# xxlong0/NeuralUDF

Measured on AMD Instinct MI355X. Metric: ray-samples/sec (train step), higher is better.
Workload: dtype f32 emulated on the 16-bit matrix pipe, f32 accumulate, f32 state / epilogues / optimizer.  Forward-order sweeps (UDF value, input gradient, colour / NeRF forward): f16x2 (x = hi + 2^-11 lo in fp16, 3 fp16 MFMA products, correction terms in their own accumulator).  Backward sweeps (tangent, adjoint

## Files before the change

### include/nudf.h

```cpp
#ifndef NUDF_H
#define NUDF_H
#include <stdint.h>

#ifdef __cplusplus
extern "C" {
#endif

int nudf_version(void);
const char* nudf_last_error(void);

enum {
  NUDF_STATUS_NONFINITE_RENDER = 1,
  NUDF_STATUS_NONFINITE_SAMPLES = 2,
  NUDF_STATUS_NONFINITE_LOSS = 4
};
int nudf_set_status_flag(int32_t* device_word);
int32_t* nudf_status_flag(void);

enum {
  NUDF_EPI_NONE = 0,
  NUDF_EPI_SOFTPLUS = 1,
  NUDF_EPI_RELU = 2,
  NUDF_EPI_MUL = 3,
  NUDF_EPI_MULMASK = 4,
// ... 375 lines not shown
  const float* seed_wrow;
  unsigned long long* dbg;
  float* absmax_out;
  const float* tile_amax_in;
  float* tile_amax_out;
  int32_t tile_scale;
  int32_t reserved0;
  NudfChainStep step[NUDF_CH_MAX_STEPS];
} NudfChain;
#if defined(__cplusplus)
static_assert(sizeof(NudfChain) <= 4096, "NudfChain travels by value: the kernel-argument segment holds 4 KB");
#endif
int nudf_mlp_chain(const NudfChain* args, void* stream);
int nudf_chain_max_steps(void);
int nudf_set_chain_t16(int on);
int nudf_pack_frag(const float* B, int ldb, int K, int N, float* out, void* stream);

#define NUDF_PACK_MAX_LAYERS 16
#define NUDF_PACK_MAX_FRAGS 4
typedef struct NudfPackFrag {
  float* dst;
  int32_t transpose;
  int32_t o0, i0;
  int32_t K, N;
  int32_t dtype;
} NudfPackFrag;
typedef struct NudfPackLayer {
  const float* v; const float* g;
  const int32_t* perm;
  float* W; float* Wt;
// ... 196 lines not shown
```

### neuraludf_amd/_lib.py

```python
from __future__ import annotations

import ctypes as C
import os

import torch

_HERE = os.path.dirname(os.path.abspath(__file__))
LIB_PATH = os.environ.get("NUDF_LIB") or os.path.join(_HERE, "libnudf.so")
ABI_VERSION = 108

c_fp = C.c_void_p
i32 = C.c_int32
f32 = C.c_float


class NudfError(RuntimeError):
    pass


class GemmNN(C.Structure):
    _fields_ = [("A", c_fp), ("lda", i32), ("B", c_fp), ("ldb", i32), ("bias", c_fp),
                ("C1", c_fp), ("ldc1", i32), ("C2", c_fp), ("ldc2", i32), ("C3", c_fp), ("ldc3", i32),
                ("X1", c_fp), ("ldx1", i32), ("X2", c_fp), ("ldx2", i32),
                ("M", i32), ("N", i32), ("K", i32), ("epi", i32), ("iparam", i32), ("scale", f32), ("xscale", f32)]
# ... 192 lines not shown

LW = dict(color_base=0, color=1, color_pixel=2, color_patch=3, igr=4, igr_ns=5, sparse=6, mask=7, color_sum=8)
LW_COUNT = 16

EPI = dict(NONE=0, SOFTPLUS=1, RELU=2, MUL=3, MULMASK=4, TANGENT=5, BWD=6, SIGMOID=7, UDFHEAD=8,
           SKIPSPLIT=9, RELU_DUAL=10, ADDMASK=11, MULSP=12)

SYMBOLS = [
    "nudf_version", "nudf_chain_max_steps", "nudf_last_error", "nudf_set_status_flag", "nudf_status_flag", "nudf_gemm_nn", "nudf_set_gemm_variant", "nudf_gemm_tn", "nudf_gemm_tn_grouped", "nudf_gemm_tn_grouped_workspace", "nudf_gemm_tn_grouped_plan", "nudf_set_tn_flags", "nudf_patch_metric", "nudf_set_tn_debug", "nudf_composite_fwd",
    "nudf_composite_bwd", "nudf_partial_sums", "nudf_composite_colour_finish", "nudf_set_composite_blocked", "nudf_upsample", "nudf_merge", "nudf_merge_points", "nudf_coarse_z", "nudf_coarse_start", "nudf_outside_z",
    "nudf_ray_points", "nudf_posenc", "nudf_posenc_vjp", "nudf_copy_cols", "nudf_add_cols",
    "nudf_udf_grad_seed", "nudf_udf_head_bwd", "nudf_signed_colsum", "nudf_sigmoid_head_bwd",
    "nudf_weightnorm_pack", "nudf_weightnorm_unpack_grad",
    "nudf_pixel_blend_fwd", "nudf_pixel_blend_bwd", "nudf_pixel_composite_fwd", "nudf_pixel_composite_bwd",
    "nudf_patch_blend_fwd", "nudf_patch_blend_bwd", "nudf_ssim_patch", "nudf_pixel_warp", "nudf_patch_warp",
    "nudf_adam_step", "nudf_adam_chunk", "nudf_mlp_chain", "nudf_set_chain_t16", "nudf_pack_frag",
    "nudf_weightnorm_pack_multi", "nudf_weightnorm_unpack_grad_multi",
    "nudf_scalars_fwd", "nudf_scalars_bwd", "nudf_l1_sum_fwd", "nudf_l1_sum_bwd",
    "nudf_sums_errors_fwd", "nudf_sums_errors_bwd", "nudf_color_loss_fwd", "nudf_color_loss_bwd",
    "nudf_gen_ray_batch", "nudf_color_loss_sums", "nudf_color_loss_finish",
    "nudf_step_loss_fwd", "nudf_step_loss_bwd", "nudf_col0_seed4",
    "nudf_blend_loss_prepare", "nudf_blend_loss_fwd", "nudf_blend_loss_bwd",
    "nudf_meshudf_classify", "nudf_meshudf_emit", "nudf_meshudf_vertices",
    "nudf_pc_tri_count", "nudf_pc_tri_emit", "nudf_pc_keys", "nudf_pc_cells", "nudf_pc_thin_round", "nudf_pc_nearest",
    "nudf_meshtopo_edges", "nudf_meshtopo_fill_count", "nudf_meshtopo_fill_emit", "nudf_meshtopo_smooth",
    "nudf_meshtopo_cc_hook", "nudf_meshtopo_cc_jump", "nudf_meshtopo_views",
]

_P, _I, _F = C.c_void_p, C.c_int, C.c_float
_ARGTYPES = {
    "nudf_gemm_nn": [C.POINTER(GemmNN), _P],
# ... 91 lines not shown
        _lib.nudf_version.restype = C.c_int
        _lib.nudf_adam_chunk.restype = C.c_int
        if _lib.nudf_version() != ABI_VERSION:
            v, _lib = _lib.nudf_version(), None
            raise NudfError(f"{LIB_PATH} is ABI version {v}, this package binds {ABI_VERSION}: rebuild with "
                            "`python -m neuraludf_amd.build --force`")
        steps = getattr(_lib, "nudf_chain_max_steps", None)
        if steps is None or int(steps()) != CH_MAX_STEPS:
            v, _lib = (None if steps is None else int(steps())), None
            raise NudfError(f"{LIB_PATH} holds {v} chain steps per launch, this package binds {CH_MAX_STEPS}: rebuild with "
                            "`python -m neuraludf_amd.build --force`")
        _bind(_lib)
        _lib.nudf_gemm_tn_grouped_workspace.restype = C.c_int64
        _lib.nudf_set_chain_t16.argtypes = [C.c_int]
        _lib.nudf_set_chain_t16.restype = C.c_int
        _lib.nudf_set_status_flag.argtypes = [C.c_void_p]
        _lib.nudf_set_status_flag.restype = C.c_int
        _lib.nudf_status_flag.argtypes = []
        _lib.nudf_status_flag.restype = C.c_void_p
    return _lib


STATUS_NONFINITE_RENDER, STATUS_NONFINITE_SAMPLES, STATUS_NONFINITE_LOSS = 1, 2, 4
_STATUS_WORDS = {}
_STATUS_BOUND = None


def bind_status(dev):
    global _STATUS_BOUND
    if dev.type != "cuda":
# ... 66 lines not shown
```

### neuraludf_amd/csrc/mlp_chain.hip

```cpp
#include "nudf_common.h"
#include "../../include/nudf.h"

#include "mlp_chain_shared.h"
#include <stdlib.h>
#include <type_traits>

template <int TM>
struct ChainSmem {
  float act[TM * CH_LD];
  float xs[TM * 3];
  float vs[TM * 3];
  float red[8];
};
#define CH_SGN_COL 288
static_assert(CH_SGN_COL < CH_LD, "the head multiplier lives in the tile's row padding");

template <int TM>
struct ChainSmem16 {
  unsigned short act[TM * CH_LD16];
  float xs[TM * 3];
  float vs[TM * 3];
  float red[8];
};

// ... 513 lines not shown
    mfmas(pa[1], b[1]);
    split(pa[0]);
    pattern();
  }
  __builtin_amdgcn_sched_barrier(0);
  if (g < G16) mfmas(pa[0], b[0]);
  }
#pragma unroll
  for (int i = 0; i < NRT; ++i)
#pragma unroll
    for (int j = 0; j < NCT; ++j)
#pragma unroll
      for (int r = 0; r < 16; ++r) acc[i][j][r] = __builtin_fmaf(acc1[i][j][r], 1.0f / 2048.0f, acc[i][j][r]);
}

typedef __bf16 ch_bf16x2 __attribute__((ext_vector_type(2)));
typedef float ch_f32x2 __attribute__((ext_vector_type(2)));
__device__ __forceinline__ void ch_p4_widen(const uint2& w, float* x) {
  x[0] = __builtin_bit_cast(float, w.x << 16);
  x[1] = __builtin_bit_cast(float, w.x & 0xffff0000u);
  x[2] = __builtin_bit_cast(float, w.y << 16);
  x[3] = __builtin_bit_cast(float, w.y & 0xffff0000u);
}
__device__ __forceinline__ void ch_p4_load(const float* X, int ld, unsigned q0, unsigned col, uint2 (&w)[4]) {
  const uint2* Xq = reinterpret_cast<const uint2*>(X) + (size_t)q0 * ld + col;
#pragma unroll
  for (int g = 0; g < 4; ++g) w[g] = Xq[(size_t)(2 * g) * ld];
}
__device__ __forceinline__ void ch_p4_store(float* C, int ld, unsigned q0, unsigned col, const float (&v)[16]) {
  uint2* Cq = reinterpret_cast<uint2*>(C) + (size_t)q0 * ld + col;
#pragma unroll
  for (int g = 0; g < 4; ++g) {
    uint2 w;
    w.x = __builtin_bit_cast(unsigned, __builtin_convertvector(ch_f32x2{v[4 * g], v[4 * g + 1]}, ch_bf16x2));
    w.y = __builtin_bit_cast(unsigned, __builtin_convertvector(ch_f32x2{v[4 * g + 2], v[4 * g + 3]}, ch_bf16x2));
    Cq[(size_t)(2 * g) * ld] = w;
  }
}

struct ChNoX3 {};
template <int EPI, bool X2IN = false, bool S16 = false, bool RT16 = false, bool T16 = false, bool HX3 = false, class X3V = ChNoX3>
__device__ __forceinline__ float ch_epilogue_tile(const NudfChainStep& st, float* act, int m0, int rtile, int ctile,
                                                 int h, int ln, f32x16 a, float (&x1)[16], bool load_x1,
                                                 const float* x2in = nullptr, const float* bias_pre = nullptr,
                                                 bool tile_bf = false, const X3V& x3in = X3V(), float tsig = 1.0f,
                                                 float tinv = 1.0f) {
  float tmax = 0.0f;
  const int col = ctile * 32 + ln;
  const bool col_ok = col < st.N;
  const unsigned colc = col_ok ? col : 0;
  const int r0 = rtile * 32 + 4 * h;
  const unsigned grow0 = (unsigned)(m0 + r0);
  float v[16], out[16];
  {
    const float bias = bias_pre ? *bias_pre : (st.bias ? st.bias[colc] : 0.0f);
#pragma unroll
    for (int r = 0; r < 16; ++r) v[r] = a[r] + bias;
  }
  if (st.r1_row) {
    const float r1c = st.r1_col[colc];
    const unsigned vo = grow0 * (unsigned)st.ldr1;
#pragma unroll
    for (int r = 0; r < 16; ++r) {
      const float rv = (st.r1_row + (size_t)CH_KOFF(r) * st.ldr1)[vo];
      tmax = fmaxf(tmax, fabsf(rv));
      v[r] += (rv * tsig) * r1c;
    }
  }
  float x2[16];
  if (CH_USES_X1(EPI) && load_x1) {
    const unsigned vo = grow0 * (unsigned)st.ldx1 + colc;
    if (S16 || (RT16 && (st.layout & NUDF_CH_P4_X1))) {
      uint2 w[4];
      ch_p4_load(st.X1, st.ldx1, (grow0 >> 2), colc, w);
// ... 128 lines not shown
#pragma unroll
          for (int r = 0; r < 16; ++r) (st.C1 + (size_t)CH_KOFF(r) * st.ldc1)[vo] = out[r];
        }
        if (st.C2 && st.N <= st.iparam) {
          const unsigned vo = grow0 * (unsigned)st.ldc2 + col;
#pragma unroll
          for (int r = 0; r < 16; ++r) (st.C2 + (size_t)CH_KOFF(r) * st.ldc2)[vo] = out[r];
        }
      } else if (st.C2) {
        const unsigned vo = grow0 * (unsigned)st.ldc2 + (col - st.iparam);
#pragma unroll
        for (int r = 0; r < 16; ++r) (st.C2 + (size_t)CH_KOFF(r) * st.ldc2)[vo] = out2[r];
      }
    }
  } else if (col_ok) {
    if (st.C1) {
      float omax = 0.0f;
#pragma unroll
      for (int r = 0; r < 16; r += 2) omax = __builtin_fmaxf(omax, __builtin_fmaxf(fabsf(out[r]), fabsf(out[r + 1])));
      tmax = __builtin_fmaxf(tmax, omax * tinv);
    }
    if (EPI == NUDF_CH_MULSP && st.iparam > 0 && col >= st.iparam) {
      if (st.C2) {
        const unsigned vo = grow0 * (unsigned)st.ldc2 + (col - st.iparam);
#pragma unroll
        for (int r = 0; r < 16; ++r) (st.C2 + (size_t)CH_KOFF(r) * st.ldc2)[vo] = out2[r] * tinv;
      }
    } else if (st.C1) {
      const unsigned vo = grow0 * (unsigned)st.ldc1 + col;
      if (S16 || (RT16 && (st.layout & NUDF_CH_P4_C1))) {
        ch_p4_store(st.C1, st.ldc1, (grow0 >> 2), (unsigned)col, out);
// ... 237 lines not shown
      for (int r = 0; r < 8; ++r) (st.C1 + (size_t)CH_KOFF(r) * st.ldc1)[vo] = out[r] * tinv;
      float omax = 0.0f;
#pragma unroll
      for (int r = 0; r < 8; r += 2) omax = __builtin_fmaxf(omax, __builtin_fmaxf(fabsf(out[r]), fabsf(out[r + 1])));
      bmax = __builtin_fmaxf(bmax, omax * tinv);
    }
    if (st.act_write) {
      float* ap = act + ((rt0 + i) * 32 + 4 * h + 16 * hf) * CH_LD + st.act_col0 + col;
#pragma unroll
      for (int r = 0; r < 8; ++r) ap[CH_KOFF(r) * CH_LD] = col_ok ? out[r] : 0.0f;
    }
  }
  return bmax;
}

template <int EPI, int MODE>
__device__ __forceinline__ float ch_epilogue(const NudfChain& p, const NudfChainStep& st, float* act, int m0, int rt0,
                                            int ct0, int nrt, int nct, int h, int ln, f32x16 (&acc)[2][2],
                                            const float (&px1)[2][2][16], const float (&bpre)[2], bool tile_bf = false,
                                            float tsig = 1.0f, float tinv = 1.0f) {
  float emax = 0.0f;
  constexpr bool ANY16 = MODE == 1 || MODE == 3 || MODE == 4, X3 = MODE == 2, T16 = MODE == 3 || MODE == 4;
  constexpr bool PF = CH_USES_X1(EPI);
  if constexpr (CH_USES_X2(EPI) && !T16) {
    if (!X3 && st.prec == 0 && nrt == 2 && !(ANY16 && (st.layout & NUDF_CH_STATE16))) {
      float(&x1)[2][2][16] = const_cast<float(&)[2][2][16]>(px1);
      if (nct == 2) ch_epilogue_seq<EPI, 2, 2>(st, act, m0, rt0, ct0, h, ln, acc, x1, bpre);
      else ch_epilogue_seq<EPI, 2, 1>(st, act, m0, rt0, ct0, h, ln, acc, x1, bpre);
      return emax;
    }
  }
// ... 73 lines not shown
            continue;
          }
        }
        ch_epilogue_tile<EPI, false, true, false, T16>(st, act, m0, rt0 + i, ct0 + j, h, ln, a, x1, true, nullptr, &bpre[j], tile_bf);
        continue;
      }
    }
    if constexpr (EPI == NUDF_CH_BWD && MODE == 1) {
      if (st.X3) {
        ch_epilogue_tile<EPI, false, false, false, T16, true>(st, act, m0, rt0 + i, ct0 + j, h, ln, a, x1, true, nullptr, &bpre[j],
                                                              tile_bf);
        continue;
      }
    }
    constexpr bool RT16 = ANY16 && (EPI == NUDF_CH_RELU || EPI == NUDF_CH_MULMASK || EPI == NUDF_CH_ADDMASK);
    emax = fmaxf(emax, ch_epilogue_tile<EPI, false, false, RT16, T16>(st, act, m0, rt0 + i, ct0 + j, h, ln, a, x1, ANY16 || X3, nullptr,
                                                                      &bpre[j], tile_bf, ChNoX3(), tsig, tinv));
  }
  return emax;
}

#ifndef NUDF_T16_WGS
#define NUDF_T16_WGS 3
#endif
#ifndef NUDF_TS_LOG2
#define NUDF_TS_LOG2 (-6)
#endif
template <int TM, int MODE>
__global__ __launch_bounds__(CH_THREADS, (MODE == 3) ? NUDF_T16_WGS : 2) void mlp_chain_kernel(NudfChain p_arg) {
  constexpr bool ANY16 = MODE == 1 || MODE == 3 || MODE == 4, X3 = MODE == 2, T16 = MODE == 3 || MODE == 4;
  (void)p_arg;
  const NudfChain& p = *(const NudfChain*)__builtin_amdgcn_kernarg_segment_ptr();
  constexpr int WMT = TM / 32;
  using Smem = typename std::conditional<T16, ChainSmem16<TM>, ChainSmem<TM>>::type;
  __shared__ __attribute__((aligned(16))) Smem sm;
  const bool tile_bf = T16 && p.step[0].prec == 2;
  const int tfmt = T16 ? (tile_bf ? 2 : 1) : 0;
  float* const act_f = reinterpret_cast<float*>(sm.act);
  const int tid = threadIdx.x;
  const int lane = tid & 63;
  const int wave = tid >> 6;
  const int h = lane >> 5, ln = lane & 31;
  const int m0 = blockIdx.x * TM;
  float amax = 0.0f;
  float tsig = 1.0f, tinv = 1.0f;
  const bool tscale = X3 && p.tile_scale != 0;
  auto wg_max = [&](float v) -> float {
#pragma unroll
    for (int off = 32; off > 0; off >>= 1) v = fmaxf(v, __shfl_xor(v, off));
    __syncthreads();
    if (lane == 0) sm.red[wave] = v;
    __syncthreads();
    float m = sm.red[0];
#pragma unroll
    for (int w = 1; w < CH_THREADS / 64; ++w) m = fmaxf(m, sm.red[w]);
    return m;
  };
  auto set_sigma = [&](float m) {
    const unsigned e = (__builtin_bit_cast(unsigned, m) >> 23) & 0xffu;
    const int se = 254 + NUDF_TS_LOG2 - (int)e;
    if (e != 0u && e != 255u && se >= 1 && se <= 254) {
// ... 5 lines not shown
    float m = 0.0f;
    for (int i = 0; i < p.n_steps; ++i) {
      const NudfChainStep& s0 = p.step[i];
      if (s0.r1_row)
        for (int e = tid; e < TM; e += CH_THREADS) m = fmaxf(m, fabsf(s0.r1_row[(size_t)min(m0 + e, p.P - 1) * s0.ldr1]));
    }
    if (p.tile_amax_in && tid < TM / 32) m = fmaxf(m, p.tile_amax_in[(m0 >> 5) + tid]);
    return m;
  };

  if (p.x) {
    for (int e = tid; e < TM * 3; e += CH_THREADS) {
      int r = m0 + e / 3;
      if (r > p.P - 1) r = p.P - 1;
      sm.xs[e] = p.x[(size_t)(r / p.x_div) * 3 + (e % 3)];
      sm.vs[e] = p.v ? p.v[(size_t)r * 3 + (e % 3)] : 0.0f;
      if (X3 && p.v && p.init == NUDF_CH_INIT_POSENC)
        amax = fmaxf(amax, fabsf(sm.vs[e] * p.pe_in_scale) * (float)(1 << (p.pe_L > 0 ? p.pe_L - 1 : 0)));
    }
  }
  if constexpr (X3) {
    if (tscale && p.init == NUDF_CH_INIT_POSENC && p.v) {
      set_sigma(wg_max(fmaxf(amax, other_seeds())));
      for (int e = tid; e < TM * 3; e += CH_THREADS) sm.vs[e] *= tsig;
    }
  }
  __syncthreads();
  if (p.init == NUDF_CH_INIT_LOAD) {
    const int k4 = p.k0 >> 2;
    for (int e = tid; e < TM * k4; e += CH_THREADS) {
      const int r = e / k4, c4 = e - r * k4;
      int gr = m0 + r;
      if (gr > p.P - 1) gr = p.P - 1;
      const f32x4 val = *reinterpret_cast<const f32x4*>(p.A0 + (size_t)gr * p.lda0 + c4 * 4);
      if constexpr (X3) amax = fmaxf(amax, fmaxf(fmaxf(fabsf(val[0]), fabsf(val[1])), fmaxf(fabsf(val[2]), fabsf(val[3]))));
      if constexpr (T16) {
        uint2 w;
        if (tile_bf) {
          w.x = (unsigned)ch_f2bf(val[0]) | ((unsigned)ch_f2bf(val[1]) << 16);
          w.y = (unsigned)ch_f2bf(val[2]) | ((unsigned)ch_f2bf(val[3]) << 16);
        } else {
          w.x = ch_f2h2(val[0], val[1]);
// ... 73 lines not shown

#ifdef NUDF_X3_CU_STAGGER
  if (X3 && gridDim.x > 256) {
    const unsigned hw = __builtin_amdgcn_s_getreg((8 << 11) | (8 << 6) | 4);
#if NUDF_X3_CU_STAGGER > 0
    const unsigned late = hw & 1u;
    for (int d = 0; d < (int)late * NUDF_X3_CU_STAGGER; ++d) __builtin_amdgcn_s_sleep(127);
#else
    const unsigned xcc = __builtin_amdgcn_s_getreg((4 << 11) | (0 << 6) | 20);
    for (int d = 0; d < (int)(xcc & 1u) * (-NUDF_X3_CU_STAGGER); ++d) __builtin_amdgcn_s_sleep(127);
#endif
  }
#endif
  unsigned long long* dbg = p.dbg ? p.dbg + ((size_t)blockIdx.x * 4 + wave) * 64 : nullptr;
  if (dbg && lane == 0) {
    dbg[0] = __builtin_amdgcn_s_getreg((31 << 11) | (0 << 6) | 4);
    dbg[1] = __builtin_amdgcn_s_memtime();
    dbg[62] = wall_clock64();
  }

  for (int si = 0; si < p.n_steps; ++si) {
    const NudfChainStep& st = p.step[si];
    if ((si + slot) & 1u) __builtin_amdgcn_s_setprio(1); else __builtin_amdgcn_s_setprio(0);
    if constexpr (X3) {
      if (st.epi == NUDF_CH_SEED) {
        int t = tid;
        asm volatile("" : "+v"(t));
        const int C = st.N;
        if (t < C) {
          const float wc = st.r1_col[t];
          float* ap = act_f + t;
          float* gp = st.C1 ? st.C1 + (size_t)m0 * st.ldc1 + t : nullptr;
#pragma unroll 4
          for (int r = 0; r < TM; ++r) {
            float s, om;
            ch_sp_derivs(ap[r * CH_LD], st.xscale, s, om);
            const float val = ap[r * CH_LD + CH_SGN_COL - t] * wc * st.scale * s;
            ap[r * CH_LD] = val;
            if (gp) gp[(size_t)r * st.ldc1] = val;
// ... 58 lines not shown
    if (nct > 0) {
      const float* arow = act_f + (rt0 * 32 + ln) * CH_LD + 4 * h;
      const f32x4* bptr = Bp + (size_t)ct0 * 64 + lane;
      const size_t bstride = (size_t)NT * 64;
      const bool pfx = !ANY16 && !X3 && CH_USES_X1(st.epi);
      ChPrefetch pf;
      pf.X1 = st.X1;
      pf.ldx1 = st.ldx1;
#pragma unroll
      for (int i = 0; i < 2; ++i)
#pragma unroll
        for (int j = 0; j < 2; ++j) {
          const int col = (ct0 + j) * 32 + ln;
          pf.vo[i][j] = (unsigned)(m0 + (rt0 + i) * 32 + 4 * h) * (unsigned)st.ldx1 + (unsigned)((col < st.N) ? col : 0);
        }
      if (X3 && st.prec == 4) {
        const float* arow16 = act_f + (rt0 * 32 + ln) * CH_LD + 8 * h;
        const uint4* bp2 = reinterpret_cast<const uint4*>(st.Bp) + (size_t)ct0 * 128 + lane;
        const size_t bstride2 = (size_t)NT * 128;
        const int G16 = st.K >> 4;
#ifdef NUDF_X2_PIPE64
        constexpr bool PIPE2 = true;
#else
        constexpr bool PIPE2 = (NUDF_X3_PIPE == 1) || (NUDF_X3_PIPE == 2 && TM == 32);
#endif
        if (nrt == 2 && nct == 2) ch_mma16x2<2, 2, PIPE2>(arow16, bp2, bstride2, G16, acc);
        else if (nrt == 2) ch_mma16x2<2, 1, PIPE2>(arow16, bp2, bstride2, G16, acc);
        else if (nct == 2) ch_mma16x2<1, 2, PIPE2>(arow16, bp2, bstride2, G16, acc);
        else ch_mma16x2<1, 1, PIPE2>(arow16, bp2, bstride2, G16, acc);
      } else if (X3 && st.prec == 3) {
// ... 30 lines not shown
        if (nrt == 2 && nct == 2) ch_mma<2, 2, true>(arow, bptr, bstride, G, acc, pf, px1);
        else if (nrt == 2) ch_mma<2, 1, true>(arow, bptr, bstride, G, acc, pf, px1);
        else if (nct == 2) ch_mma<1, 2, true>(arow, bptr, bstride, G, acc, pf, px1);
        else ch_mma<1, 1, true>(arow, bptr, bstride, G, acc, pf, px1);
      } else {
        if (nrt == 2 && nct == 2) ch_mma<2, 2, false>(arow, bptr, bstride, G, acc, pf, px1);
        else if (nrt == 2) ch_mma<2, 1, false>(arow, bptr, bstride, G, acc, pf, px1);
        else if (nct == 2) ch_mma<1, 2, false>(arow, bptr, bstride, G, acc, pf, px1);
        else ch_mma<1, 1, false>(arow, bptr, bstride, G, acc, pf, px1);
      }
    }
    if (dbg && lane == 0 && si < 14) dbg[2 + 4 * si] = __builtin_amdgcn_s_memtime();
    __syncthreads();
    if (dbg && lane == 0 && si < 14) dbg[3 + 4 * si] = __builtin_amdgcn_s_memtime();

    if (nct > 0) {
      switch (st.epi) {
        case NUDF_CH_SOFTPLUS: ch_epilogue<NUDF_CH_SOFTPLUS, MODE>(p, st, act_f, m0, rt0, ct0, nrt, nct, h, ln, acc, px1, bpre, tile_bf, tsig, tinv); break;
        case NUDF_CH_NONE: { const float em = ch_epilogue<NUDF_CH_NONE, MODE>(p, st, act_f, m0, rt0, ct0, nrt, nct, h, ln, acc, px1, bpre, tile_bf, tsig, tinv); if constexpr (X3) amax = fmaxf(amax, em); } break;
        case NUDF_CH_MULSP: { const float em = ch_epilogue<NUDF_CH_MULSP, MODE>(p, st, act_f, m0, rt0, ct0, nrt, nct, h, ln, acc, px1, bpre, tile_bf, tsig, tinv); if constexpr (X3) amax = fmaxf(amax, em); } break;
        case NUDF_CH_TANGENT:
          if constexpr (MODE != 3) ch_epilogue<NUDF_CH_TANGENT, MODE>(p, st, act_f, m0, rt0, ct0, nrt, nct, h, ln, acc, px1, bpre, tile_bf, tsig, tinv);
          break;
        case NUDF_CH_BWD: { const float em = ch_epilogue<NUDF_CH_BWD, MODE>(p, st, act_f, m0, rt0, ct0, nrt, nct, h, ln, acc, px1, bpre, tile_bf, tsig, tinv); if constexpr (X3) amax = fmaxf(amax, em); } break;
        case NUDF_CH_RELU: ch_epilogue<NUDF_CH_RELU, MODE>(p, st, act_f, m0, rt0, ct0, nrt, nct, h, ln, acc, px1, bpre, tile_bf, tsig, tinv); break;
        case NUDF_CH_SIGMOIDN: ch_epilogue<NUDF_CH_SIGMOIDN, MODE>(p, st, act_f, m0, rt0, ct0, nrt, nct, h, ln, acc, px1, bpre, tile_bf, tsig, tinv); break;
        case NUDF_CH_MULMASK: { const float em = ch_epilogue<NUDF_CH_MULMASK, MODE>(p, st, act_f, m0, rt0, ct0, nrt, nct, h, ln, acc, px1, bpre, tile_bf, tsig, tinv); if constexpr (X3) amax = fmaxf(amax, em); } break;
        case NUDF_CH_ADDMASK: { const float em = ch_epilogue<NUDF_CH_ADDMASK, MODE>(p, st, act_f, m0, rt0, ct0, nrt, nct, h, ln, acc, px1, bpre, tile_bf, tsig, tinv); if constexpr (X3) amax = fmaxf(amax, em); } break;
        case NUDF_CH_RELUADD: ch_epilogue<NUDF_CH_RELUADD, MODE>(p, st, act_f, m0, rt0, ct0, nrt, nct, h, ln, acc, px1, bpre, tile_bf, tsig, tinv); break;
        default: ch_epilogue<NUDF_CH_UDFHEAD, MODE>(p, st, act_f, m0, rt0, ct0, nrt, nct, h, ln, acc, px1, bpre, tile_bf, tsig, tinv); break;
      }
    }
    if (dbg && lane == 0 && si < 14) dbg[4 + 4 * si] = __builtin_amdgcn_s_memtime();
    if (st.pe_tail_col >= 0) {
      __syncthreads();
      const int pe_end = st.pe_tail_col + 3 * (2 * p.pe_L + 1);
      ch_write_pe<TM>(sm, p, m0, st.pe_tail_col, st.pe_tail_scale, st.pe_dst, st.ld_pe, st.pe_tail_col,
                      min((pe_end + 15) & ~15, 288), (st.layout & NUDF_CH_STATE16) != 0, tfmt, tinv);
    }
    __syncthreads();
    if (dbg && lane == 0 && si < 14) dbg[5 + 4 * si] = __builtin_amdgcn_s_memtime();
  }
  if (dbg && lane == 0) dbg[63] = wall_clock64();
  if constexpr (X3) {
    if (p.tile_amax_out) {
      const float m = wg_max(amax);
      if (tid < TM / 32) p.tile_amax_out[(m0 >> 5) + tid] = m;
    }
    if (p.absmax_out) {
#pragma unroll
      for (int off = 32; off > 0; off >>= 1) amax = fmaxf(amax, __shfl_xor(amax, off));
      if (lane == 0 && amax > 0.0f && amax < 3.0e38f) atomicMax(reinterpret_cast<unsigned*>(p.absmax_out), __builtin_bit_cast(unsigned, amax));
    }
  }
}

int nudf_chain_rows_class(const NudfChain& p, bool allow_blocked = false);
int nudf_mlp_chain_rows_launch(const NudfChain& p, int cls, hipStream_t st);
int nudf_mlp_chain_tq_launch(const NudfChain& p, int cls, hipStream_t st, int force_pair = 0);
// ... 15 lines not shown
  return mode;
}

static int g_chain_t16 = -1;
static bool nudf_chain_t16_enabled() {
  if (g_chain_t16 < 0) {
    const char* e = getenv("NUDF_CHAIN_T16");
    g_chain_t16 = (e && e[0] == '0') ? 0 : 1;
  }
  return g_chain_t16 != 0;
}
extern "C" int nudf_set_chain_t16(int on) {
  const int old = nudf_chain_t16_enabled() ? 1 : 0;
  g_chain_t16 = on ? 1 : 0;
  return old;
}

extern "C" int nudf_chain_max_steps(void) { return NUDF_CH_MAX_STEPS; }

extern "C" int nudf_mlp_chain(const NudfChain* args, void* stream) {
  const NudfChain& p = *args;
  if (p.P <= 0 || p.n_steps <= 0) return 0;
  bool bad = p.n_steps > NUDF_CH_MAX_STEPS || (p.k0 & 3) || p.k0 > 288 || p.x_div < 1;
  bool fused = false;
  for (int i = 0; i < p.n_steps && !bad; ++i) {
    const NudfChainStep& s = p.step[i];
    if (s.epi == NUDF_CH_SEED) {
      bad = i == 0 || i + 1 >= p.n_steps || p.step[i - 1].epi != NUDF_CH_UDFHEAD || p.step[i - 1].act_write || !s.r1_col ||
            s.N <= 0 || s.N > 256 || p.step[i + 1].K < s.N || p.step[i + 1].K > ((s.N + 15) & ~15) || (s.C1 && s.ldc1 < s.N) ||
            s.layout || s.pe_tail_col >= 0 || s.X3 || s.row_w || p.tile_scale || p.tile_amax_in || p.tile_amax_out || p.absmax_out;
// ... 92 lines not shown
  }
  if (!roww && !fused && (p.tile_rows == 66 || (p.tile_rows == 0 && p.P > 256 * 64 && nudf_chain_quad_mode() > 0))) {
    const int cls = nudf_chain_rows_class(p);
    if (cls >= 0 && (p.tile_rows == 66 || cls <= 1 || nudf_chain_quad_mode() >= 2)) return nudf_mlp_chain_tq_launch(p, cls, st);
  }
  if (!roww && p.tile_rows == 0 && p.P >= 32768 && !any16 && !any3 && nudf_chain_pair_mode() >= 2) {
    const int cls = nudf_chain_rows_class(p);
    if (cls >= 0) return nudf_mlp_chain_tq_launch(p, cls, st);
  }
  bool t16 = any16 && !roww && nudf_chain_t16_enabled();
  bool t16_tangent = false;
  for (int i = 0; i < p.n_steps && t16; ++i) {
    t16 = (p.step[i].prec == 1 || p.step[i].prec == 2) && p.step[i].prec == p.step[0].prec;
    t16_tangent = t16_tangent || p.step[i].epi == NUDF_CH_TANGENT || p.step[i].X3 != nullptr;
  }
  if (p.tile_rows == 32 || (p.tile_rows != 64 && p.P <= 256 * 64)) {
    if (any3) hipLaunchKernelGGL((mlp_chain_kernel<32, 2>), dim3((p.P + 31) / 32), dim3(CH_THREADS), 0, st, p);
    else if (any16) hipLaunchKernelGGL((mlp_chain_kernel<32, 1>), dim3((p.P + 31) / 32), dim3(CH_THREADS), 0, st, p);
    else hipLaunchKernelGGL((mlp_chain_kernel<32, 0>), dim3((p.P + 31) / 32), dim3(CH_THREADS), 0, st, p);
  } else {
    if (any3) hipLaunchKernelGGL((mlp_chain_kernel<64, 2>), dim3((p.P + 63) / 64), dim3(CH_THREADS), 0, st, p);
    else if (t16 && t16_tangent) hipLaunchKernelGGL((mlp_chain_kernel<64, 4>), dim3((p.P + 63) / 64), dim3(CH_THREADS), 0, st, p);
    else if (t16) hipLaunchKernelGGL((mlp_chain_kernel<64, 3>), dim3((p.P + 63) / 64), dim3(CH_THREADS), 0, st, p);
    else if (any16) hipLaunchKernelGGL((mlp_chain_kernel<64, 1>), dim3((p.P + 63) / 64), dim3(CH_THREADS), 0, st, p);
    else hipLaunchKernelGGL((mlp_chain_kernel<64, 0>), dim3((p.P + 63) / 64), dim3(CH_THREADS), 0, st, p);
  }
  NUDF_CHECK_LAUNCH("nudf_mlp_chain");
  return 0;
}

__global__ void pack_frag_kernel(const float* __restrict__ B, int ldb, int K, int N, int NT, int total,
                                 float* __restrict__ out) {
  const int idx = blockIdx.x * blockDim.x + threadIdx.x;
  if (idx >= total) return;
  const int j = idx & 3, lane = (idx >> 2) & 63, gt = idx >> 8;
  const int T = gt % NT, g = gt / NT;
// ... 14 lines not shown
```

### neuraludf_amd/mlp.py

```python
from __future__ import annotations

import math
from typing import List, Optional

import ctypes as C

import torch

from . import _lib
import os

from ._lib import CH, CH_INIT, CH_MAX_STEPS, EPI, Chain, GemmNN, GemmTN, call, ptr


def pad32(n: int) -> int:
    return (n + 31) // 32 * 32


def pad_rows(P: int) -> int:
    return (P + 63) // 64 * 64


def _buf(P, width, dev, zero=None, dtype=torch.float32, blocked=False):
    if blocked:
# ... 390 lines not shown
        if CHAIN_DEBUG is not None:
            self.c.dbg = ptr(CHAIN_DEBUG)
        if PROFILE is not None:
            _timed("mlp_chain", self.flops, lambda: call("nudf_mlp_chain", self.c), self._label(), self.nbytes, self.xflops)
        else:
            call("nudf_mlp_chain", self.c)
        if memo_ok and sig is not None and len(slots) == len(ptrs):
            ms = _CHAIN_MEMO.setdefault(mkey, [])
            if len(ms) >= 4:
                ms.pop(0)
            ms.append([sig, self.c, slots, ptrs])
            if len(_CHAIN_MEMO) > 512:
                _CHAIN_MEMO.clear()
        self.keep = []

    def _label(self):
        P, e = self.c.P, set(self.epis)
        x1 = bool(e & {"MULSP", "TANGENT", "BWD", "MULMASK", "ADDMASK"})
        x2 = bool(e & {"TANGENT", "BWD", "ADDMASK", "RELUADD"})
        pair = int(os.environ.get("NUDF_CHAIN_PAIR", "0"))
        if self.c.tile_rows == 130 or ((self.blocked or self.c.tile_rows == 66) and pair >= 1 and P >= 32768):
            kern = "mlp_chain_pair_kernel<%d>" % (2 if x2 else (1 if x1 else 0))
        elif self.c.tile_rows == 0 and pair >= 2 and P >= 32768 and PRECISION == "fp32":
            kern = "mlp_chain_pair_kernel<%d>" % (2 if x2 else (1 if x1 else 0))
        elif self.blocked or self.c.tile_rows == 66:
            kern = "mlp_chain_tq_kernel<%d>" % (2 if x2 else (1 if x1 else 0))
        elif self.c.tile_rows == 128:
            kern = "mlp_chain_rows_kernel"
        else:
            mode = {"fp32": 0, "mixed16": 1, "bf16x3": 2}[PRECISION]
            t32 = self.c.tile_rows == 32 or (self.c.tile_rows != 64 and P <= 256 * 64)
            roww = any(self.c.step[i].row_w for i in range(self.n))
            if mode == 1 and not t32 and not roww and _chain_t16_now():
                precs = {int(self.c.step[i].prec) for i in range(self.n)}
                if len(precs) == 1 and precs <= {1, 2}:
                    x3 = any(self.c.step[i].X3 for i in range(self.n))
                    mode = 4 if ("TANGENT" in e or x3) else 3
            kern = "mlp_chain_kernel<%d, %d>" % (32 if t32 else 64, mode)
        sweep = ("udf-forward+input-gradient" if "SEED" in e
                 else "tangent" if ("TANGENT" in e or ("MULSP" in e and self.init == "POSENC")) else "adjoint" if "BWD" in e
                 else "input-gradient" if "MULSP" in e
                 else "relu-backward" if e & {"MULMASK", "ADDMASK"} else "udf-forward" if "SOFTPLUS" in e
                 else "relu-forward")
        return "%s %s P=%d" % (kern, sweep, P)


def _chain_t16_now():
    L = _lib.lib()
    old = int(L.nudf_set_chain_t16(1))
    L.nudf_set_chain_t16(old)
    return bool(old)


TN_DETERMINISTIC = True
_TN_WS = {}


def _tn_workspace(g, dev):
    need = int(_lib.lib().nudf_gemm_tn_grouped_workspace(C.byref(g)))
# ... 1369 lines not shown
```

Baseline: 20.40 million.

## Add lean forward-only chain kernel instantiation with ring-buffered f16x2 MMA

Adds a compile-time forward-only family of the split-precision MLP chain kernel. It strips tangent, seed, tile-scale, r1 and C1 handling from pure forward chains (posenc init, softplus/none/udfhead epilogues), which should cut register pressure and branching. It also introduces a multi-stage ring-buffered B-fragment prefetch for the f16x2 MFMA loop, with configurable depth. The lean kernel is chosen at launch by host-side eligibility checks and is on by default, with an env var to disable it. The risk is larger code size and a mismatch between the host predicate and the features the kernel actually supports.

Result: no change. 20.41 million, median of 5 (+0.1%).

```diff
diff --git a/include/nudf.h b/include/nudf.h
--- a/include/nudf.h
+++ b/include/nudf.h
@@ -413,6 +413,7 @@
 int nudf_mlp_chain(const NudfChain* args, void* stream);
 int nudf_chain_max_steps(void);
 int nudf_set_chain_t16(int on);
+int nudf_set_chain_lean(int on);
 int nudf_pack_frag(const float* B, int ldb, int K, int N, float* out, void* stream);
 
 #define NUDF_PACK_MAX_LAYERS 16
diff --git a/neuraludf_amd/_lib.py b/neuraludf_amd/_lib.py
--- a/neuraludf_amd/_lib.py
+++ b/neuraludf_amd/_lib.py
@@ -230,7 +230,7 @@
     "nudf_weightnorm_pack", "nudf_weightnorm_unpack_grad",
     "nudf_pixel_blend_fwd", "nudf_pixel_blend_bwd", "nudf_pixel_composite_fwd", "nudf_pixel_composite_bwd",
     "nudf_patch_blend_fwd", "nudf_patch_blend_bwd", "nudf_ssim_patch", "nudf_pixel_warp", "nudf_patch_warp",
-    "nudf_adam_step", "nudf_adam_chunk", "nudf_mlp_chain", "nudf_set_chain_t16", "nudf_pack_frag",
+    "nudf_adam_step", "nudf_adam_chunk", "nudf_mlp_chain", "nudf_set_chain_t16", "nudf_set_chain_lean", "nudf_pack_frag",
     "nudf_weightnorm_pack_multi", "nudf_weightnorm_unpack_grad_multi",
     "nudf_scalars_fwd", "nudf_scalars_bwd", "nudf_l1_sum_fwd", "nudf_l1_sum_bwd",
     "nudf_sums_errors_fwd", "nudf_sums_errors_bwd", "nudf_color_loss_fwd", "nudf_color_loss_bwd",
@@ -352,6 +352,8 @@
         _lib.nudf_gemm_tn_grouped_workspace.restype = C.c_int64
         _lib.nudf_set_chain_t16.argtypes = [C.c_int]
         _lib.nudf_set_chain_t16.restype = C.c_int
+        _lib.nudf_set_chain_lean.argtypes = [C.c_int]
+        _lib.nudf_set_chain_lean.restype = C.c_int
         _lib.nudf_set_status_flag.argtypes = [C.c_void_p]
         _lib.nudf_set_status_flag.restype = C.c_int
         _lib.nudf_status_flag.argtypes = []
diff --git a/neuraludf_amd/csrc/mlp_chain.hip b/neuraludf_amd/csrc/mlp_chain.hip
--- a/neuraludf_amd/csrc/mlp_chain.hip
+++ b/neuraludf_amd/csrc/mlp_chain.hip
@@ -551,6 +551,105 @@
       for (int r = 0; r < 16; ++r) acc[i][j][r] = __builtin_fmaf(acc1[i][j][r], 1.0f / 2048.0f, acc[i][j][r]);
 }
 
+#ifndef NUDF_FWD_RING32
+#define NUDF_FWD_RING32 3
+#endif
+#ifndef NUDF_FWD_RING64
+#define NUDF_FWD_RING64 1
+#endif
+template <int NRT, int NCT, bool PIPE, int D>
+__device__ __forceinline__ void ch_mma16x2_ring(const float* __restrict__ arow, const uint4* __restrict__ bptr, size_t bstride2,
+                                                int G16, f32x16 (&acc)[2][2]) {
+  constexpr int R = D + 1;
+  constexpr int U = (R % 2 == 0) ? R : 2 * R;
+  f32x4 raw[NRT][2];
+  f16x8 pa[2][NRT][2];
+  uint4 b[R][NCT][2];
+  f32x16 acc1[NRT][NCT];
+#pragma unroll
+  for (int i = 0; i < NRT; ++i)
+#pragma unroll
+    for (int j = 0; j < NCT; ++j)
+#pragma unroll
+      for (int r = 0; r < 16; ++r) acc1[i][j][r] = 0.0f;
+  auto lda = [&](int g) {
+#pragma unroll
+    for (int i = 0; i < NRT; ++i) {
+      raw[i][0] = *reinterpret_cast<const f32x4*>(arow + i * 32 * CH_LD + g * 16);
+      raw[i][1] = *reinterpret_cast<const f32x4*>(arow + i * 32 * CH_LD + g * 16 + 4);
+    }
+  };
+  auto ldb = [&](uint4 (&bb)[NCT][2], int g) {
+    const uint4* bq = bptr + (size_t)g * bstride2;
+#pragma unroll
+    for (int j = 0; j < NCT; ++j)
+#pragma unroll
+      for (int pl = 0; pl < 2; ++pl) bb[j][pl] = bq[j * 128 + pl * 64];
+  };
+  auto split = [&](f16x8 (&q)[NRT][2]) {
+#pragma unroll
+    for (int i = 0; i < NRT; ++i) ch_split2(raw[i][0], raw[i][1], q[i][0], q[i][1]);
+  };
+  auto mfmas = [&](const f16x8 (&q)[NRT][2], const uint4 (&bb)[NCT][2]) {
+#pragma unroll
+    for (int t = 0; t < 3; ++t)
+#pragma unroll
+      for (int i = 0; i < NRT; ++i)
+#pragma unroll
+        for (int j = 0; j < NCT; ++j) {
+          const f16x8 av = (t == 1) ? q[i][1] : q[i][0];
+          const f16x8 bv = __builtin_bit_cast(f16x8, (t == 0) ? bb[j][1] : bb[j][0]);
+          if (t < 2) acc1[i][j] = __builtin_amdgcn_mfma_f32_32x32x16_f16(av, bv, acc1[i][j], 0, 0, 0);
+          else acc[i][j] = __builtin_amdgcn_mfma_f32_32x32x16_f16(av, bv, acc[i][j], 0, 0, 0);
+        }
+  };
+  auto pattern = [&]() {
+    if constexpr (PIPE) {
+      __builtin_amdgcn_sched_group_barrier(0x100, 2 * NRT, 0);
+      __builtin_amdgcn_sched_group_barrier(0x020, 2 * NCT, 0);
+#pragma unroll
+      for (int m = 0; m < 3 * NRT * NCT; ++m) {
+        __builtin_amdgcn_sched_group_barrier(0x008, 1, 0);
+        __builtin_amdgcn_sched_group_barrier(0x002, (32 * NRT + 3 * NRT * NCT - 1) / (3 * NRT * NCT), 0);
+      }
+    }
+  };
+  const int gl = G16 - 1;
+  lda(0);
+#pragma unroll
+  for (int d = 0; d < D; ++d) ldb(b[d], min(d, gl));
+  split(pa[0]);
+#define CH_RING_STEP(u)                                             \
+  {                                                                 \
+    __builtin_amdgcn_sched_barrier(0);                              \
+    lda(min(g + (u) + 1, gl));                                      \
+    ldb(b[((u) + D) % R], min(g + (u) + D, gl));                    \
+    if constexpr (!PIPE) __builtin_amdgcn_sched_barrier(0);         \
+    mfmas(pa[(u) & 1], b[(u) % R]);                                 \
+    split(pa[((u) + 1) & 1]);                                       \
+    pattern();                                                      \
+  }
+  int g = 0;
+#pragma unroll 1
+  for (; g + U <= G16; g += U) {
+#pragma unroll
+    for (int u = 0; u < U; ++u) CH_RING_STEP(u)
+  }
+#pragma unroll
+  for (int u = 0; u < U - 1; ++u) {
+    if (g + u >= G16) break;
+    CH_RING_STEP(u)
+  }
+#undef CH_RING_STEP
+  __builtin_amdgcn_sched_barrier(0);
+#pragma unroll
+  for (int i = 0; i < NRT; ++i)
+#pragma unroll
+    for (int j = 0; j < NCT; ++j)
+#pragma unroll
+      for (int r = 0; r < 16; ++r) acc[i][j][r] = __builtin_fmaf(acc1[i][j][r], 1.0f / 2048.0f, acc[i][j][r]);
+}
+
 typedef __bf16 ch_bf16x2 __attribute__((ext_vector_type(2)));
 typedef float ch_f32x2 __attribute__((ext_vector_type(2)));
 __device__ __forceinline__ void ch_p4_widen(const uint2& w, float* x) {
@@ -576,7 +675,8 @@
 }
 
 struct ChNoX3 {};
-template <int EPI, bool X2IN = false, bool S16 = false, bool RT16 = false, bool T16 = false, bool HX3 = false, class X3V = ChNoX3>
+template <int EPI, bool X2IN = false, bool S16 = false, bool RT16 = false, bool T16 = false, bool HX3 = false, class X3V = ChNoX3,
+          bool LEAN = false>
 __device__ __forceinline__ float ch_epilogue_tile(const NudfChainStep& st, float* act, int m0, int rtile, int ctile,
                                                  int h, int ln, f32x16 a, float (&x1)[16], bool load_x1,
                                                  const float* x2in = nullptr, const float* bias_pre = nullptr,
@@ -594,7 +694,7 @@
 #pragma unroll
     for (int r = 0; r < 16; ++r) v[r] = a[r] + bias;
   }
-  if (st.r1_row) {
+  if (!LEAN && st.r1_row) {
     const float r1c = st.r1_col[colc];
     const unsigned vo = grow0 * (unsigned)st.ldr1;
 #pragma unroll
@@ -753,7 +853,7 @@
       }
     }
   } else if (col_ok) {
-    if (st.C1) {
+    if (!LEAN && st.C1) {
       float omax = 0.0f;
 #pragma unroll
       for (int r = 0; r < 16; r += 2) omax = __builtin_fmaxf(omax, __builtin_fmaxf(fabsf(out[r]), fabsf(out[r + 1])));
@@ -1021,7 +1121,7 @@
   return bmax;
 }
 
-template <int EPI, int MODE>
+template <int EPI, int MODE, bool LEAN = false>
 __device__ __forceinline__ float ch_epilogue(const NudfChain& p, const NudfChainStep& st, float* act, int m0, int rt0,
                                             int ct0, int nrt, int nct, int h, int ln, f32x16 (&acc)[2][2],
                                             const float (&px1)[2][2][16], const float (&bpre)[2], bool tile_bf = false,
@@ -1125,8 +1225,9 @@
       }
     }
     constexpr bool RT16 = ANY16 && (EPI == NUDF_CH_RELU || EPI == NUDF_CH_MULMASK || EPI == NUDF_CH_ADDMASK);
-    emax = fmaxf(emax, ch_epilogue_tile<EPI, false, false, RT16, T16>(st, act, m0, rt0 + i, ct0 + j, h, ln, a, x1, ANY16 || X3, nullptr,
-                                                                      &bpre[j], tile_bf, ChNoX3(), tsig, tinv));
+    emax = fmaxf(emax, ch_epilogue_tile<EPI, false, false, RT16, T16, false, ChNoX3, LEAN>(st, act, m0, rt0 + i, ct0 + j, h, ln, a, x1,
+                                                                                           ANY16 || X3, nullptr, &bpre[j], tile_bf,
+                                                                                           ChNoX3(), tsig, tinv));
   }
   return emax;
 }
@@ -1137,9 +1238,13 @@
 #ifndef NUDF_TS_LOG2
 #define NUDF_TS_LOG2 (-6)
 #endif
-template <int TM, int MODE>
+#define CH_FAM_ALL 0
+#define CH_FAM_FWD 1
+template <int TM, int MODE, int FAM = CH_FAM_ALL>
 __global__ __launch_bounds__(CH_THREADS, (MODE == 3) ? NUDF_T16_WGS : 2) void mlp_chain_kernel(NudfChain p_arg) {
   constexpr bool ANY16 = MODE == 1 || MODE == 3 || MODE == 4, X3 = MODE == 2, T16 = MODE == 3 || MODE == 4;
+  constexpr bool FWD = FAM == CH_FAM_FWD;
+  static_assert(!FWD || MODE == 2, "the forward-only family is an instantiation of the split-mode kernel");
   (void)p_arg;
   const NudfChain& p = *(const NudfChain*)__builtin_amdgcn_kernarg_segment_ptr();
   constexpr int WMT = TM / 32;
@@ -1155,7 +1260,7 @@
   const int m0 = blockIdx.x * TM;
   float amax = 0.0f;
   float tsig = 1.0f, tinv = 1.0f;
-  const bool tscale = X3 && p.tile_scale != 0;
+  const bool tscale = X3 && !FWD && p.tile_scale != 0;
   auto wg_max = [&](float v) -> float {
 #pragma unroll
     for (int off = 32; off > 0; off >>= 1) v = fmaxf(v, __shfl_xor(v, off));
@@ -1191,18 +1296,21 @@
       int r = m0 + e / 3;
       if (r > p.P - 1) r = p.P - 1;
       sm.xs[e] = p.x[(size_t)(r / p.x_div) * 3 + (e % 3)];
-      sm.vs[e] = p.v ? p.v[(size_t)r * 3 + (e % 3)] : 0.0f;
-      if (X3 && p.v && p.init == NUDF_CH_INIT_POSENC)
+      sm.vs[e] = (!FWD && p.v) ? p.v[(size_t)r * 3 + (e % 3)] : 0.0f;
+      if (X3 && !FWD && p.v && p.init == NUDF_CH_INIT_POSENC)
         amax = fmaxf(amax, fabsf(sm.vs[e] * p.pe_in_scale) * (float)(1 << (p.pe_L > 0 ? p.pe_L - 1 : 0)));
     }
   }
-  if constexpr (X3) {
+  if constexpr (X3 && !FWD) {
     if (tscale && p.init == NUDF_CH_INIT_POSENC && p.v) {
       set_sigma(wg_max(fmaxf(amax, other_seeds())));
       for (int e = tid; e < TM * 3; e += CH_THREADS) sm.vs[e] *= tsig;
     }
   }
   __syncthreads();
+  if constexpr (FWD) {
+    ch_write_pe<TM>(sm, p, m0, 0, 1.0f, p.G0, p.ldg0, 0, p.k0, false, tfmt, 1.0f);
+  } else
   if (p.init == NUDF_CH_INIT_LOAD) {
     const int k4 = p.k0 >> 2;
     for (int e = tid; e < TM * k4; e += CH_THREADS) {
@@ -1306,6 +1414,7 @@
 #endif
   unsigned long long* dbg = p.dbg ? p.dbg + ((size_t)blockIdx.x * 4 + wave) * 64 : nullptr;
   if (dbg && lane == 0) {
+    dbg[61] = FAM;
     dbg[0] = __builtin_amdgcn_s_getreg((31 << 11) | (0 << 6) | 4);
     dbg[1] = __builtin_amdgcn_s_memtime();
     dbg[62] = wall_clock64();
@@ -1314,7 +1423,7 @@
   for (int si = 0; si < p.n_steps; ++si) {
     const NudfChainStep& st = p.step[si];
     if ((si + slot) & 1u) __builtin_amdgcn_s_setprio(1); else __builtin_amdgcn_s_setprio(0);
-    if constexpr (X3) {
+    if constexpr (X3 && !FWD) {
       if (st.epi == NUDF_CH_SEED) {
         int t = tid;
         asm volatile("" : "+v"(t));
@@ -1403,6 +1512,25 @@
           const int col = (ct0 + j) * 32 + ln;
           pf.vo[i][j] = (unsigned)(m0 + (rt0 + i) * 32 + 4 * h) * (unsigned)st.ldx1 + (unsigned)((col < st.N) ? col : 0);
         }
+      if constexpr (FWD) {
+        if (st.prec == 4) {
+          const float* arow16 = act_f + (rt0 * 32 + ln) * CH_LD + 8 * h;
+          const uint4* bp2 = reinterpret_cast<const uint4*>(st.Bp) + (size_t)ct0 * 128 + lane;
+          const size_t bstride2 = (size_t)NT * 128;
+          const int G16 = st.K >> 4;
+          constexpr bool PIPE2 = (NUDF_X3_PIPE == 1) || (NUDF_X3_PIPE == 2 && TM == 32);
+          constexpr int RD = (TM == 32) ? NUDF_FWD_RING32 : NUDF_FWD_RING64;
+          if (nrt == 2 && nct == 2) ch_mma16x2_ring<2, 2, PIPE2, RD>(arow16, bp2, bstride2, G16, acc);
+          else if (nrt == 2) ch_mma16x2_ring<2, 1, PIPE2, RD>(arow16, bp2, bstride2, G16, acc);
+          else if (nct == 2) ch_mma16x2_ring<1, 2, PIPE2, RD>(arow16, bp2, bstride2, G16, acc);
+          else ch_mma16x2_ring<1, 1, PIPE2, RD>(arow16, bp2, bstride2, G16, acc);
+        } else {
+          if (nrt == 2 && nct == 2) ch_mma<2, 2, false>(arow, bptr, bstride, G, acc, pf, px1);
+          else if (nrt == 2) ch_mma<2, 1, false>(arow, bptr, bstride, G, acc, pf, px1);
+          else if (nct == 2) ch_mma<1, 2, false>(arow, bptr, bstride, G, acc, pf, px1);
+          else ch_mma<1, 1, false>(arow, bptr, bstride, G, acc, pf, px1);
+        }
+      } else
       if (X3 && st.prec == 4) {
         const float* arow16 = act_f + (rt0 * 32 + ln) * CH_LD + 8 * h;
         const uint4* bp2 = reinterpret_cast<const uint4*>(st.Bp) + (size_t)ct0 * 128 + lane;
@@ -1463,6 +1591,15 @@
     __syncthreads();
     if (dbg && lane == 0 && si < 14) dbg[3 + 4 * si] = __builtin_amdgcn_s_memtime();
 
+    if constexpr (FWD) {
+      if (nct > 0) {
+        switch (st.epi) {
+          case NUDF_CH_SOFTPLUS: ch_epilogue<NUDF_CH_SOFTPLUS, MODE, true>(p, st, act_f, m0, rt0, ct0, nrt, nct, h, ln, acc, px1, bpre); break;
+          case NUDF_CH_NONE: ch_epilogue<NUDF_CH_NONE, MODE, true>(p, st, act_f, m0, rt0, ct0, nrt, nct, h, ln, acc, px1, bpre); break;
+          default: ch_epilogue<NUDF_CH_UDFHEAD, MODE, true>(p, st, act_f, m0, rt0, ct0, nrt, nct, h, ln, acc, px1, bpre); break;
+        }
+      }
+    } else
     if (nct > 0) {
       switch (st.epi) {
         case NUDF_CH_SOFTPLUS: ch_epilogue<NUDF_CH_SOFTPLUS, MODE>(p, st, act_f, m0, rt0, ct0, nrt, nct, h, ln, acc, px1, bpre, tile_bf, tsig, tinv); break;
@@ -1485,13 +1622,13 @@
       __syncthreads();
       const int pe_end = st.pe_tail_col + 3 * (2 * p.pe_L + 1);
       ch_write_pe<TM>(sm, p, m0, st.pe_tail_col, st.pe_tail_scale, st.pe_dst, st.ld_pe, st.pe_tail_col,
-                      min((pe_end + 15) & ~15, 288), (st.layout & NUDF_CH_STATE16) != 0, tfmt, tinv);
+                      min((pe_end + 15) & ~15, 288), !FWD && (st.layout & NUDF_CH_STATE16) != 0, tfmt, tinv);
     }
     __syncthreads();
     if (dbg && lane == 0 && si < 14) dbg[5 + 4 * si] = __builtin_amdgcn_s_memtime();
   }
   if (dbg && lane == 0) dbg[63] = wall_clock64();
-  if constexpr (X3) {
+  if constexpr (X3 && !FWD) {
     if (p.tile_amax_out) {
       const float m = wg_max(amax);
       if (tid < TM / 32) p.tile_amax_out[(m0 >> 5) + tid] = m;
@@ -1537,6 +1674,34 @@
   const int old = nudf_chain_t16_enabled() ? 1 : 0;
   g_chain_t16 = on ? 1 : 0;
   return old;
+}
+
+static int g_chain_lean = -1;
+static bool nudf_chain_lean_enabled() {
+  if (g_chain_lean < 0) {
+    const char* e = getenv("NUDF_CHAIN_LEAN");
+    g_chain_lean = (e && e[0] == '0') ? 0 : 1;
+  }
+  return g_chain_lean != 0;
+}
+extern "C" int nudf_set_chain_lean(int on) {
+  const int old = nudf_chain_lean_enabled() ? 1 : 0;
+  g_chain_lean = on ? 1 : 0;
+  return old;
+}
+static bool nudf_chain_fwd_family(const NudfChain& p) {
+  if (p.init != NUDF_CH_INIT_POSENC || !p.x || p.v || p.pe_jvp || p.init_state16 || p.tile_scale || p.tile_amax_in ||
+      p.tile_amax_out || p.absmax_out || (p.tile_rows != 0 && p.tile_rows != 32 && p.tile_rows != 64))
+    return false;
+  bool split = false;
+  for (int i = 0; i < p.n_steps; ++i) {
+    const NudfChainStep& s = p.step[i];
+    if ((s.epi != NUDF_CH_SOFTPLUS && s.epi != NUDF_CH_NONE && s.epi != NUDF_CH_UDFHEAD) || (s.prec != 4 && s.prec != 0) ||
+        s.X2 || s.X3 || s.r1_row || s.r1_col || s.row_w || s.layout)
+      return false;
+    split = split || s.prec == 4;
+  }
+  return split;
 }
 
 extern "C" int nudf_chain_max_steps(void) { return NUDF_CH_MAX_STEPS; }
@@ -1659,12 +1824,15 @@
     t16 = (p.step[i].prec == 1 || p.step[i].prec == 2) && p.step[i].prec == p.step[0].prec;
     t16_tangent = t16_tangent || p.step[i].epi == NUDF_CH_TANGENT || p.step[i].X3 != nullptr;
   }
+  const bool lean = any3 && !any16 && nudf_chain_lean_enabled() && nudf_chain_fwd_family(p);
   if (p.tile_rows == 32 || (p.tile_rows != 64 && p.P <= 256 * 64)) {
-    if (any3) hipLaunchKernelGGL((mlp_chain_kernel<32, 2>), dim3((p.P + 31) / 32), dim3(CH_THREADS), 0, st, p);
+    if (any3 && lean) hipLaunchKernelGGL((mlp_chain_kernel<32, 2, CH_FAM_FWD>), dim3((p.P + 31) / 32), dim3(CH_THREADS), 0, st, p);
+    else if (any3) hipLaunchKernelGGL((mlp_chain_kernel<32, 2>), dim3((p.P + 31) / 32), dim3(CH_THREADS), 0, st, p);
     else if (any16) hipLaunchKernelGGL((mlp_chain_kernel<32, 1>), dim3((p.P + 31) / 32), dim3(CH_THREADS), 0, st, p);
     else hipLaunchKernelGGL((mlp_chain_kernel<32, 0>), dim3((p.P + 31) / 32), dim3(CH_THREADS), 0, st, p);
   } else {
-    if (any3) hipLaunchKernelGGL((mlp_chain_kernel<64, 2>), dim3((p.P + 63) / 64), dim3(CH_THREADS), 0, st, p);
+    if (any3 && lean) hipLaunchKernelGGL((mlp_chain_kernel<64, 2, CH_FAM_FWD>), dim3((p.P + 63) / 64), dim3(CH_THREADS), 0, st, p);
+    else if (any3) hipLaunchKernelGGL((mlp_chain_kernel<64, 2>), dim3((p.P + 63) / 64), dim3(CH_THREADS), 0, st, p);
     else if (t16 && t16_tangent) hipLaunchKernelGGL((mlp_chain_kernel<64, 4>), dim3((p.P + 63) / 64), dim3(CH_THREADS), 0, st, p);
     else if (t16) hipLaunchKernelGGL((mlp_chain_kernel<64, 3>), dim3((p.P + 63) / 64), dim3(CH_THREADS), 0, st, p);
     else if (any16) hipLaunchKernelGGL((mlp_chain_kernel<64, 1>), dim3((p.P + 63) / 64), dim3(CH_THREADS), 0, st, p);
diff --git a/neuraludf_amd/mlp.py b/neuraludf_amd/mlp.py
--- a/neuraludf_amd/mlp.py
+++ b/neuraludf_amd/mlp.py
@@ -428,6 +428,18 @@
                 _CHAIN_MEMO.clear()
         self.keep = []
 
+    def _fwd_family(self):
+        c = self.c
+        if (c.init != CH_INIT["POSENC"] or not c.x or c.v or c.pe_jvp or c.init_state16 or c.tile_scale or c.tile_amax_in
+                or c.tile_amax_out or c.absmax_out or c.tile_rows not in (0, 32, 64)):
+            return False
+        ok = {CH["SOFTPLUS"], CH["NONE"], CH["UDFHEAD"]}
+        steps = [c.step[i] for i in range(self.n)]
+        if any(s.epi not in ok or s.prec not in (0, 4) or s.X2 or s.X3 or s.r1_row or s.r1_col or s.row_w or s.layout
+               for s in steps):
+            return False
+        return any(s.prec == 4 for s in steps)
+
     def _label(self):
         P, e = self.c.P, set(self.epis)
         x1 = bool(e & {"MULSP", "TANGENT", "BWD", "MULMASK", "ADDMASK"})
@@ -451,12 +463,25 @@
                     x3 = any(self.c.step[i].X3 for i in range(self.n))
                     mode = 4 if ("TANGENT" in e or x3) else 3
             kern = "mlp_chain_kernel<%d, %d>" % (32 if t32 else 64, mode)
+            if mode == 2 and self._fwd_family() and _chain_lean_now():
+                kern = "mlp_chain_kernel<%d, 2, FWD>" % (32 if t32 else 64)
         sweep = ("udf-forward+input-gradient" if "SEED" in e
                  else "tangent" if ("TANGENT" in e or ("MULSP" in e and self.init == "POSENC")) else "adjoint" if "BWD" in e
                  else "input-gradient" if "MULSP" in e
                  else "relu-backward" if e & {"MULMASK", "ADDMASK"} else "udf-forward" if "SOFTPLUS" in e
                  else "relu-forward")
         return "%s %s P=%d" % (kern, sweep, P)
+
+
+def _chain_lean_now():
+    L = _lib.lib()
+    old = int(L.nudf_set_chain_lean(1))
+    L.nudf_set_chain_lean(old)
+    return bool(old)
+
+
+def set_chain_lean(on):
+    return bool(_lib.lib().nudf_set_chain_lean(1 if on else 0))
 
 
 def _chain_t16_now():
```
